# wsakobe/CylinderTag

Measured on AMD Instinct MI355X. Metric: frames/sec detect() 1920x1080, higher is better.
Workload: dtype u8; 1 GPU; synthetic 1920x1080 random-stripe frames, 4096 per step over 1 GPU(s), 4 planted CTag_2f12c markers each, detect(img,5,true,5), inputs resident in HBM; frames_per_gpu=4096, chunk=4096, parallelism=frames sharded, dp1, gather=none (1 GPU)

## Files before the change

cylindertag_amd/csrc/ctag_math.h:

```cpp
#pragma once
#include <stdint.h>

#if defined(__HIPCC__)
#define CTM_HD __host__ __device__ __forceinline__
#else
#define CTM_HD static inline
#endif

namespace ctm {

CTM_HD double bits_to_f64(uint64_t u) { double d; __builtin_memcpy(&d, &u, 8); return d; }
CTM_HD uint64_t f64_to_bits(double d) { uint64_t u; __builtin_memcpy(&u, &d, 8); return u; }
CTM_HD float bits_to_f32(uint32_t u) { float f; __builtin_memcpy(&f, &u, 4); return f; }
CTM_HD uint32_t f32_to_bits(float f) { uint32_t u; __builtin_memcpy(&u, &f, 4); return u; }

CTM_HD double fabs64(double x) { return bits_to_f64(f64_to_bits(x) & 0x7fffffffffffffffULL); }
CTM_HD float fabs32(float x) { return bits_to_f32(f32_to_bits(x) & 0x7fffffffu); }
CTM_HD bool isnan64(double x) { return x != x; }

CTM_HD double atan64(double x) {
    const double hi0 = 4.63647609000806093515e-01, hi1 = 7.85398163397448278999e-01,
                 hi2 = 9.82793723247329054082e-01, hi3 = 1.57079632679489655800e+00;
    const double lo0 = 2.26987774529616870924e-17, lo1 = 3.06161699786838301793e-17,
                 lo2 = 1.39033110312309984516e-17, lo3 = 6.12323399573676603587e-17;
// ... 102 lines not shown
    const int q = rem_pio2_64(x, &r);
    switch (q) {
        case 0: return ksin64(r);
        case 1: return kcos64(r);
        case 2: return -ksin64(r);
        default: return -kcos64(r);
    }
}
CTM_HD double cos64(double x) {
    if (fabs64(x) <= 7.85398163397448278999e-01) return kcos64(x);
    double r;
    const int q = rem_pio2_64(x, &r);
    switch (q) {
        case 0: return kcos64(r);
        case 1: return -ksin64(r);
        case 2: return -kcos64(r);
        default: return ksin64(r);
    }
}

CTM_HD void sincos64(double x, double* s, double* c) {
    double r = x;
    int q = 0;
    if (!(fabs64(x) <= 7.85398163397448278999e-01)) q = rem_pio2_64(x, &r);
    const double ks = ksin64(r), kc = kcos64(r);
    const double sv = (q & 1) ? kc : ks, cv = (q & 1) ? ks : kc;
    *s = (q & 2) ? -sv : sv;
    *c = ((q + 1) & 2) ? -cv : cv;
}

CTM_HD double exp64(double x) {
    const double T[32] = {
        1.00000000000000000e+00, 1.02189714865411663e+00, 1.04427378242741375e+00, 1.06714040067682370e+00,
        1.09050773266525769e+00, 1.11438674259589243e+00, 1.13878863475669156e+00, 1.16372485877757748e+00,
        1.18920711500272103e+00, 1.21524735998046896e+00, 1.24185781207348400e+00, 1.26905095719173322e+00,
        1.29683955465100964e+00, 1.32523664315974132e+00, 1.35425554693689265e+00, 1.38390988196383202e+00,
        1.41421356237309515e+00, 1.44518080697704665e+00, 1.47682614593949935e+00, 1.50916442759342284e+00,
        1.54221082540794074e+00, 1.57598084510788650e+00, 1.61049033194925428e+00, 1.64575547815396495e+00,
        1.68179283050742900e+00, 1.71861929812247793e+00, 1.75625216037329945e+00, 1.79470907500310717e+00,
        1.83400808640934243e+00, 1.87416763411029996e+00, 1.91520656139714740e+00, 1.95714412417540018e+00};
    const double inv = 4.61662413084468283841e+01;
    const double c_hi = 2.16608493865351192653e-02;
    const double c_lo = 5.96317165397058656257e-12;
    if (isnan64(x)) return x;
    if (x > 709.0) return bits_to_f64(0x7ff0000000000000ULL);
    if (x < -708.0) return 0.0;
    const double fn = __builtin_floor(x * inv + 0.5);
    const int n = (int)fn;
    const int j = n & 31, k = (n - j) / 32;
    const double r = (x - fn * c_hi) - fn * c_lo;
    double p = 1.3888888888888889e-03;
    p = p * r + 8.3333333333333332e-03;
    p = p * r + 4.1666666666666664e-02;
    p = p * r + 1.6666666666666666e-01;
    p = p * r + 0.5;
    p = p * r + 1.0;
    const double e = p * r + 1.0;
    const double scale = bits_to_f64((uint64_t)(k + 1023) << 52);
    return (T[j] * e) * scale;
}

CTM_HD double log64(double x) {
    const double ln2_hi = 6.93147180369123816490e-01, ln2_lo = 1.90821492927058770002e-10;
    const double Lg1 = 6.666666666666735130e-01, Lg2 = 3.999999999940941908e-01, Lg3 = 2.857142874366239149e-01,
                 Lg4 = 2.222219843214978396e-01, Lg5 = 1.818357216161805012e-01, Lg6 = 1.531383769920937332e-01,
                 Lg7 = 1.479819860511658591e-01;
    uint64_t u = f64_to_bits(x);
    uint32_t hx = (uint32_t)(u >> 32);
    int k = 0;
    if (hx < 0x00100000u || (hx >> 31)) {
        if ((u << 1) == 0) return -bits_to_f64(0x7ff0000000000000ULL);
        if (hx >> 31) return bits_to_f64(0x7ff8000000000000ULL);
        k -= 54;
        x = x * 18014398509481984.0;
        u = f64_to_bits(x);
        hx = (uint32_t)(u >> 32);
    } else if (hx >= 0x7ff00000u) {
        return x;
    } else if (u == 0x3ff0000000000000ULL) {
        return 0.0;
    }
    hx += 0x3ff00000u - 0x3fe6a09eu;
    k += (int)(hx >> 20) - 0x3ff;
    hx = (hx & 0x000fffffu) + 0x3fe6a09eu;
    const double f = bits_to_f64(((uint64_t)hx << 32) | (u & 0xffffffffULL)) - 1.0;
    const double hfsq = 0.5 * f * f;
    const double s = f / (2.0 + f);
    const double z = s * s;
    const double w = z * z;
    const double t1 = w * (Lg2 + w * (Lg4 + w * Lg6));
    const double t2 = z * (Lg1 + w * (Lg3 + w * (Lg5 + w * Lg7)));
    const double R = t2 + t1;
    const double dk = (double)k;
    return s * (hfsq + R) + dk * ln2_lo - hfsq + f + dk * ln2_hi;
}

CTM_HD double acos64(double t) {
    if (t >= 1.0) return 0.0;
    if (t <= -1.0) return 3.1415926535897931160E+00;
    return 2.0 * atan2_64(__builtin_sqrt(1.0 - t), __builtin_sqrt(1.0 + t));
}

constexpr float kAcosBelowTenMilli = 0.99995005130767822266f;

CTM_HD float atan2_32(float y, float x) { return (float)atan2_64((double)y, (double)x); }
CTM_HD float sin32(float x) { return (float)sin64((double)x); }
CTM_HD float cos32(float x) { return (float)cos64((double)x); }
CTM_HD void sincos32(float x, float* s, float* c) {
    double sd, cd;
    sincos64((double)x, &sd, &cd);
    *s = (float)sd;
    *c = (float)cd;
}
CTM_HD float exp32(float x) {
    if (x != x) return x;
    if (x < -87.0f) return 0.0f;
    if (x > 88.0f) return bits_to_f32(0x7f800000u);
    const float k = __builtin_rintf(x * 1.44269502162933349609375f);
    const float r = (x - k * 0.693145751953125f) - k * 1.428606765330187045037746429443359375e-06f;
    float p = 1.3933733571320772171020508e-03f;
    p = p * r + 8.3632357418537139892578125e-03f;
    p = p * r + 4.1666463017463684082031250e-02f;
    p = p * r + 1.6666576266288757324218750e-01f;
    p = p * r + 0.5f;
    const float e = (p * (r * r) + r) + 1.0f;
    return e * bits_to_f32((uint32_t)((int)k + 127) << 23);
}
CTM_HD float exp32_nonpos(float x) {
    if (x < -87.0f) return 0.0f;
    const float k = __builtin_rintf(x * 1.44269502162933349609375f);
    const float r = (x - k * 0.693145751953125f) - k * 1.428606765330187045037746429443359375e-06f;
    float p = 1.3933733571320772171020508e-03f;
    p = p * r + 8.3632357418537139892578125e-03f;
    p = p * r + 4.1666463017463684082031250e-02f;
    p = p * r + 1.6666576266288757324218750e-01f;
    p = p * r + 0.5f;
    const float e = (p * (r * r) + r) + 1.0f;
#if defined(__HIP_DEVICE_COMPILE__)
    return __builtin_amdgcn_ldexpf(e, (int)k);
#else
    return e * bits_to_f32((uint32_t)((int)k + 127) << 23);
#endif
}
CTM_HD bool exp32_k_is_zero(float x) { return x * 1.44269502162933349609375f >= -0.5f; }
CTM_HD float exp32_nonpos_k0(float x) {
    const float r = x;
    float p = 1.3933733571320772171020508e-03f;
    p = p * r + 8.3632357418537139892578125e-03f;
    p = p * r + 4.1666463017463684082031250e-02f;
    p = p * r + 1.6666576266288757324218750e-01f;
    p = p * r + 0.5f;
    return (p * (r * r) + r) + 1.0f;
}
struct Recip64 {
    double d, r;
};
CTM_HD Recip64 recip64(double d) {
    Recip64 R;
    R.d = d;
#if defined(__HIP_DEVICE_COMPILE__)
    double r = __builtin_amdgcn_rcp(d);
    r = __builtin_fma(r, __builtin_fma(-d, r, 1.0), r);
    r = __builtin_fma(r, __builtin_fma(-d, r, 1.0), r);
    R.r = r;
#else
    R.r = 0.0;
#endif
    return R;
}
CTM_HD double div64(double a, const Recip64& R) {
#if defined(__HIP_DEVICE_COMPILE__)
    const double q = a * R.r;
    return __builtin_fma(__builtin_fma(-R.d, q, a), R.r, q);
#else
    return a / R.d;
#endif
}
CTM_HD float sqrt32(float x) { return __builtin_sqrtf(x); }
CTM_HD double sqrt64(double x) { return __builtin_sqrt(x); }
CTM_HD float round32(float x) {
    const float ax = fabs32(x);
    if (!(ax < 8388608.0f)) return x;
    float r = __builtin_floorf(ax);
    if (ax - r >= 0.5f) r += 1.0f;
    return (f32_to_bits(x) >> 31) ? -r : r;
}

CTM_HD float fast_atan2_deg(float y, float x) {
    const float s = (float)(180.0 / 3.1415926535897932384626433832795);
    const float p1 = 0.9997878412794807f * s, p3 = -0.3258083974640975f * s,
                p5 = 0.1555786518463281f * s, p7 = -0.04432655554792128f * s;
    const float eps = (float)2.2204460492503131e-16;
    const float ax = fabs32(x), ay = fabs32(y);
    float a, c, c2;
    if (ax >= ay) {
        c = ay / (ax + eps);
        c2 = c * c;
        a = (((p7 * c2 + p5) * c2 + p3) * c2 + p1) * c;
    } else {
        c = ax / (ay + eps);
        c2 = c * c;
        a = 90.0f - (((p7 * c2 + p5) * c2 + p3) * c2 + p1) * c;
    }
    if (x < 0) a = 180.0f - a;
    if (y < 0) a = 360.0f - a;
    return a;
}

CTM_HD bool solve2x2(float a00, float a01, float a10, float a11, float b0, float b1, float& x0, float& x1) {
    double d = (double)a00 * a11 - (double)a01 * a10;
    if (d == 0.) return false;
    d = 1. / d;
    const float t = (float)(((double)b0 * a11 - (double)b1 * a01) * d);
    x1 = (float)(((double)b1 * a00 - (double)b0 * a10) * d);
    x0 = t;
    return true;
}

}
```

cylindertag_amd/csrc/k_quad.hip:

```cpp
#include "ctag_internal.h"
#include "ctag_math.h"
#include "ctag_wave.h"
#include <cstdio>
#include <type_traits>
#include <cstdlib>

namespace ctag {

struct QuadPtrs {
    const uint16_t* labels;
    const int32_t* tile_base;
    const int32_t* root_of;
    const int32_t* ncand;
    const Candidate* cand;
    QuadOut* quads;
    uint32_t* frame_flags;
    int32_t* line_count;
    int32_t* clp_used;
    uint32_t* cl_pool;
    LineDesc* line_desc;
    int32_t* line_sorted;
    int32_t* line_long;
    float* line_fit;
    CandAux* cand_aux;
    const uint8_t* pick_table;
    const uint16_t* pick_table16;
    const int32_t* pool_tile;
    const int32_t* member_head;
    const int32_t* member_next;
    int32_t* npacks;
    uint32_t* packs;
    uint32_t* pack_order;
    int32_t* npacks2;
    uint32_t* packs2;
    uint32_t* pack_order2;
    int32_t* npacks1;
    uint32_t* packs1;
    uint32_t* pack_order1;
    int32_t* ntotal1;
    unsigned long long* stamps;
    float thr_line, thr_expand, rac;
    int c2_far, c2_near;
    int cand_cap, line_cap;
    uint32_t cl_cap;
    float expand_eps;
    const uint64_t* mask;
    int mask_words;
};
static QuadPtrs quad_ptrs(const ChunkPlan& pl, const Workspace& ws, unsigned long long* stamps) {
    QuadPtrs P{};
    P.labels = ws.labels, P.tile_base = ws.tile_base, P.root_of = ws.root_of, P.ncand = ws.ncand, P.cand = ws.cand, P.quads = ws.quads, P.frame_flags = ws.frame_flags;
    P.line_count = ws.line_count, P.clp_used = ws.clp_used, P.cl_pool = ws.cl_pool, P.line_desc = ws.line_desc, P.line_sorted = ws.line_sorted, P.line_long = ws.line_long;
    P.line_fit = ws.line_fit, P.cand_aux = ws.cand_aux, P.pick_table = ws.pick_table, P.pick_table16 = ws.pick_table16;
    P.pool_tile = ws.pool_tile, P.member_head = ws.member_head, P.member_next = ws.member_next;
    P.npacks = ws.npacks, P.packs = ws.packs, P.pack_order = ws.pack_order, P.stamps = stamps;
    P.npacks2 = ws.npacks2, P.packs2 = ws.packs2, P.pack_order2 = ws.pack_order2;
    P.npacks1 = ws.npacks1, P.packs1 = ws.packs1, P.pack_order1 = ws.pack_order1, P.ntotal1 = ws.ntotal1;
    P.thr_line = ws.kp.thr_line, P.thr_expand = ws.kp.thr_expand, P.rac = ws.kp.rac, P.c2_far = ws.kp.c2_far, P.c2_near = ws.kp.c2_near, P.expand_eps = ws.kp.expand_eps;
    P.cand_cap = ws.cand_cap, P.line_cap = ws.line_cap, P.cl_cap = ws.cl_cap;
    P.mask = pl.fused ? reinterpret_cast<const uint64_t*>(ws.half) : nullptr, P.mask_words = ws.g.hcols >> 6;
    return P;
}

__device__ __forceinline__ uint32_t pack_xy(int x, int y) { return (uint32_t)x | ((uint32_t)y << 16); }
__device__ __forceinline__ int ux(uint32_t p) { return (int)(p & 0xffffu); }
__device__ __forceinline__ int uy(uint32_t p) { return (int)(p >> 16); }

__device__ __forceinline__ void moments_to_line(double x, double y, double x2, double y2, double xy, double w, float* line) {
    const ctm::Recip64 W = ctm::recip64(w);
    x = ctm::div64(x, W);
    y = ctm::div64(y, W);
    x2 = ctm::div64(x2, W);
    y2 = ctm::div64(y2, W);
    xy = ctm::div64(xy, W);
    const double dx2 = x2 - x * x, dy2 = y2 - y * y, dxy = xy - x * y;
    const float t = (float)ctm::atan2_64(2 * dxy, dx2 - dy2) / 2;
    double sn, cs;
    ctm::sincos64(t, &sn, &cs);
    line[0] = (float)cs;
    line[1] = (float)sn;
    line[2] = (float)x;
    line[3] = (float)y;
}

struct CvRng {
    uint64_t state;
    __device__ unsigned next() {
        state = (uint64_t)(unsigned)state * 4164903690U + (unsigned)(state >> 32);
        return (unsigned)state;
    }
};

#ifndef CTAG_WCAP
#define CTAG_WCAP 16
#endif
#ifndef CTAG_WUNROLL
#define CTAG_WUNROLL 2
#endif
#define CTAG_PRAGMA_(x) _Pragma(#x)
#define CTAG_PRAGMA(x) CTAG_PRAGMA_(x)
constexpr int kWCap = CTAG_WCAP;
struct GlobalPts {
    const uint32_t* p;
    __device__ __forceinline__ float2 operator()(int j) const {
        const uint32_t v = p[j];
        return make_float2((float)ux(v), (float)uy(v));
    }
};
struct LdsPts {
    const float2* p;
    __device__ __forceinline__ float2 operator()(int j) const { return p[j]; }
};
struct LdsPackedPts {
    const uint32_t* p;
    __device__ __forceinline__ float2 operator()(int j) const {
        const uint32_t v = p[j];
        return make_float2((float)ux(v), (float)uy(v));
    }
};
struct TablePicks {
    const uint8_t* t;
    __device__ __forceinline__ int operator()(int i) const { return t[i]; }
};
struct ListPicks {
    const uint16_t* t;
    __device__ __forceinline__ int operator()(int i) const { return t[i]; }
};
struct AllPicks {
    __device__ __forceinline__ int operator()(int i) const { return i; }
};
struct RestartResult {
    float line[4];
    double err;
};
__device__ __forceinline__ RestartResult restart_result(const float* res, int rstride) {
    RestartResult r;
    for (int q = 0; q < 4; q++) r.line[q] = res[q * rstride];
    const uint64_t lo = ctm::f32_to_bits(res[4 * rstride]), hi = ctm::f32_to_bits(res[5 * rstride]);
    r.err = ctm::bits_to_f64(lo | (hi << 32));
    return r;
}
template <class Pts, class Picks>
__device__ __forceinline__ void welsch_first_fit(const Pts pts, const Picks picks, int npick, float* line) {
    double x = 0, y = 0, x2 = 0, y2 = 0, xy = 0, w = 0;
    for (int i = 0; i < npick; i++) {
        const float2 p = pts(picks(i));
        const float px = p.x, py = p.y;
        x += px;
        y += py;
        x2 += px * px;
        y2 += py * py;
        xy += px * py;
        w += 1.f;
    }
    moments_to_line(x, y, x2, y2, xy, w, line);
}
struct WeightTrips {
    unsigned fast = 0, general = 0;
};
template <bool COUNT>
__device__ __forceinline__ float welsch_weight(float a, WeightTrips& trips) {
    const bool fast = wave_all(ctm::exp32_k_is_zero(a));
    if constexpr (COUNT) {
        const bool first = (int)__lane_id() == __ffsll((unsigned long long)__ballot(1)) - 1;
        trips.fast += first && fast ? 1u : 0u;
        trips.general += first && !fast ? 1u : 0u;
    }
    if (fast) return ctm::exp32_nonpos_k0(a);
    return ctm::exp32_nonpos(a);
}
template <int WS, bool COUNT, class Pts>
__device__ __forceinline__ bool welsch_rounds(const Pts pts, int n, double EPS, float* line, double& err, int it0, int it_stop, bool resume, float* wc, int ncache, WeightTrips& trips) {
    float prev[4] = {0.f, 0.f, 0.f, 0.f};
    const float c = 1 / 2.9846f;
#ifdef CTAG_WELSCH_MINERR_IN_LOOP
    double berr = 1.7976931348623157e308;
    float bl[4] = {0.f, 0.f, 0.f, 0.f};
#define CTAG_WELSCH_HAND_ON()       \
    do {                            \
        for (int q = 0; q < 4; q++) line[q] = bl[q]; \
        err = berr;                 \
    } while (0)
#else
#define CTAG_WELSCH_HAND_ON() do { } while (0)
#endif
    for (int it = it0; it < 30; it++) {
        if (it > 0 && !(resume && it == it0)) {
            const float t = line[0] * prev[0] + line[1] * prev[1];
            if (t >= ctm::kAcosBelowTenMilli) {
                const float dx = ctm::fabs32(line[2] - prev[2]);
                const float dy = ctm::fabs32(line[3] - prev[3]);
                const float d = dx > dy ? dx : dy;
                if (d < 0.01f) {
                    CTAG_WELSCH_HAND_ON();
                    return true;
                }
            }
        }
        if (it == it_stop) return false;
        const float lx = line[2], ly = line[3], nx = line[1], ny = -line[0];
        double sum_w = 0;
        err = 0;
        float2 pn0 = pts(min(0, n - 1));
        for (int j = 0; j < ncache; j++) {
            const float2 p = pn0;
            pn0 = pts(j + 1);
            const float x = p.x - lx, y = p.y - ly;
            const float r = ctm::fabs32(nx * x + ny * y);
            err += r;
            const float wj = welsch_weight<COUNT>(-r * r * c * c, trips);
            wc[j * WS] = wj;
            sum_w += wj;
        }
        float2 pn1 = pts(min(ncache, n - 1));
        for (int j = ncache; j < n; j++) {
            const float2 p = pn1;
            pn1 = pts(j + 1);
            const float x = p.x - lx, y = p.y - ly;
            const float r = ctm::fabs32(nx * x + ny * y);
            err += r;
            sum_w += welsch_weight<COUNT>(-r * r * c * c, trips);
        }
#ifdef CTAG_WELSCH_MINERR_IN_LOOP
        if (err < berr) {
            berr = err;
            for (int q = 0; q < 4; q++) bl[q] = line[q];
            if (err < EPS) return true;
        }
#else
        if (err < EPS) return true;
#endif
        double x = 0, y = 0, x2 = 0, y2 = 0, xy = 0, w = 0;
        if (ctm::fabs64(sum_w) > 1.1920928955078125e-07) {
            const double inv = 1. / sum_w;
            float2 pn2 = pts(min(0, n - 1));
            CTAG_PRAGMA(unroll CTAG_WUNROLL)
            for (int j = 0; j < ncache; j++) {
                const float2 p = pn2;
                pn2 = pts(j + 1);
                const float px = p.x, py = p.y;
                const float wj = (float)(wc[j * WS] * inv);
                x += wj * px;
                y += wj * py;
                x2 += wj * px * px;
                y2 += wj * py * py;
                xy += wj * px * py;
                w += wj;
            }
            float2 pn3 = pts(min(ncache, n - 1));
            for (int j = ncache; j < n; j++) {
                const float2 p = pn3;
                pn3 = pts(j + 1);
                const float px = p.x, py = p.y;
                const float r = ctm::fabs32(nx * (px - lx) + ny * (py - ly));
                const float wj = (float)(welsch_weight<COUNT>(-r * r * c * c, trips) * inv);
                x += wj * px;
                y += wj * py;
                x2 += wj * px * px;
                y2 += wj * py * py;
                xy += wj * px * py;
                w += wj;
            }
        } else {
            float2 pn4 = pts(min(0, n - 1));
            for (int j = 0; j < n; j++) {
                const float2 p = pn4;
                pn4 = pts(j + 1);
                const float px = p.x, py = p.y;
                x += px;
                y += py;
                x2 += px * px;
                y2 += py * py;
                xy += px * py;
                w += 1.f;
            }
        }
        prev[0] = line[0];
        prev[1] = line[1];
        prev[2] = line[2];
        prev[3] = line[3];
        moments_to_line(x, y, x2, y2, xy, w, line);
    }
    CTAG_WELSCH_HAND_ON();
    return true;
}
#undef CTAG_WELSCH_HAND_ON
__device__ __forceinline__ void restart_store(float* res, int rstride, const float* line, double err) {
    for (int q = 0; q < 4; q++) res[q * rstride] = line[q];
    const uint64_t eb = ctm::f64_to_bits(err);
    res[4 * rstride] = ctm::bits_to_f32((uint32_t)eb);
    res[5 * rstride] = ctm::bits_to_f32((uint32_t)(eb >> 32));
}
template <int WS, bool COUNT, class Pts, class Picks>
__device__ __forceinline__ void welsch_restart(const Pts pts, int n, const Picks picks, int npick, double EPS, float* res, int rstride, float* wc, WeightTrips& trips) {
    float line[4];
    double err = 0;
    welsch_first_fit(pts, picks, npick, line);
    (void)welsch_rounds<WS, COUNT>(pts, n, EPS, line, err, 0, 30, false, wc, min(n, kWCap), trips);
    restart_store(res, rstride, line, err);
}

#ifndef CTAG_PACK_WORDS
#define CTAG_PACK_WORDS 5120
#endif
#ifndef CTAG_PACK_WAVES
#define CTAG_PACK_WAVES 2
#endif
constexpr int kPackWords = CTAG_PACK_WORDS;
#ifndef CTAG_PACK_WAVES_P2
#define CTAG_PACK_WAVES_P2 4
#endif
constexpr int kPackWordsSmall = 2560, kPackWavesSmall = 4, kPackWavesSmallP2 = CTAG_PACK_WAVES_P2;
constexpr int kUnwind = 8;
constexpr int kWaveWords = 8192;
constexpr int kWaveWordsMax = 36864;
__host__ __device__ __forceinline__ int pack_points(int w, int h) { return min(2 * (w + h), w * h) + 1; }
__host__ __device__ __forceinline__ int pack_need(int w, int h) {
    const int C = pack_points(w, h);
    return ((w + 1) & ~1) + 2 * h + 2 * C + 4;
}
__host__ __device__ __forceinline__ int need2(int n) { return 2 * ((n + 1) & ~1); }
__host__ __device__ __forceinline__ int need1(int w, int h, int nt) { return (w + h + 2 * nt + 6) & ~1; }
constexpr int kScanWords = 2048;
__host__ __device__ __forceinline__ int scan_need(int w, int h) { return w + 3 * h + 4; }
constexpr int kMaskScanWords = 512, kMaskScanWordsLarge = 2048;
__host__ __device__ __forceinline__ int mask_scan_need(int w, int h) { return h * ((w + 31) / 32 + 1); }
__host__ __device__ __forceinline__ bool pack_big(int x_min, int w, int h, int big_points, int pack_words, int scan_words = 0) {
    (void)x_min;
    return pack_need(w, h) > pack_words || pack_points(w, h) > big_points || (scan_words > 0 && scan_need(w, h) > scan_words) ||
           (scan_words < 0 && mask_scan_need(w, h) > -scan_words);
}

struct CornerPre {
    float x, y, dis, ang;
};

__device__ __forceinline__ int pack_rank_sort(const int* s_key, uint16_t* s_ord, int n, int tid, int nt) {
    int neg = 0;
    for (int i = tid; i < n; i += nt) {
        const int ki = s_key[i];
        int rank = 0;
        for (int j = 0; j < n; j++) {
            const int kj = s_key[j];
            rank += (kj > ki || (kj == ki && j < i)) ? 1 : 0;
        }
        s_ord[rank] = (uint16_t)i;
        neg += ki < 0 ? 1 : 0;
    }
    return neg;
}
template <class KeyOf, class ValOf>
__device__ __forceinline__ int pack_counting_sort(int* s_cnt, uint32_t* out, int n, int tid, int nt, KeyOf key_of, ValOf val_of) {
    constexpr int kB = kLdsCand;
    auto bucket_of = [&](int key) { return key < 0 ? kB : kB - 1 - min(key, kB - 1); };
    for (int b = tid; b <= kB; b += nt) s_cnt[b] = 0;
    __syncthreads();
    for (int i = tid; i < n; i += nt) atomicAdd(&s_cnt[bucket_of(key_of(i))], 1);
    __syncthreads();
    if (tid == 0) {
        int run = 0;
        for (int b = 0; b <= kB; b++) {
            const int v = s_cnt[b];
            s_cnt[b] = run;
            run += v;
        }
        s_cnt[kB + 1] = run;
    }
    __syncthreads();
    const int first_neg = s_cnt[kB];
    __syncthreads();
    for (int i = tid; i < n; i += nt) out[atomicAdd(&s_cnt[bucket_of(key_of(i))], 1)] = val_of(i);
    __syncthreads();
    return first_neg;
}
template <class NeedOf>
__device__ __forceinline__ int build_packs(uint32_t* packs, int npacked, int max_per_pack, int pack_words, int tid, NeedOf need_of) {
    int np = 0, first = -1, cnt = 0, words = 0;
    for (int r0 = 0; r0 < npacked; r0 += 64) {
        const int r = r0 + tid;
        const int need = r < npacked ? need_of(r) : 0;
        const int m = min(64, npacked - r0);
        for (int k = 0; k < m; k++) {
            const int nk = __builtin_amdgcn_readlane(need, k);
            if (cnt > 0 && (cnt == max_per_pack || words + nk > pack_words)) {
                if (tid == 0) packs[np] = (uint32_t)first | ((uint32_t)cnt << 24);
                np++;
                cnt = 0;
                words = 0;
            }
            if (cnt == 0) first = r0 + k;
            cnt++;
            words += nk;
        }
    }
    if (cnt > 0) {
        if (tid == 0) packs[np] = (uint32_t)first | ((uint32_t)cnt << 24);
        np++;
    }
    return np;
}

__global__ __launch_bounds__(1024) void k_pack(QuadPtrs P, int nframes, int max_per_pack, int big_points, int pack_words, int scan_words) {
    __shared__ int s_key[kLdsCand + 2];
    __shared__ int s_need[kLdsCand];
    __shared__ uint16_t s_ord[kLdsCand];
    const int frame = blockIdx.x;
    if (frame >= nframes) return;
    const int tid = threadIdx.x, nt = blockDim.x;
    const int nc = min(P.ncand[frame], P.cand_cap);
    const Candidate* cand = P.cand + (size_t)frame * P.cand_cap;
    uint32_t* order = P.pack_order + (size_t)frame * P.cand_cap;
    uint32_t* packs = P.packs + (size_t)frame * P.cand_cap;
    auto key_of = [&](const Candidate& c) {
        const int w = c.x_max - c.x_min + 1, h = c.y_max - c.y_min + 1;
        return pack_big(c.x_min, w, h, big_points, pack_words, scan_words) ? -1 : pack_points(w, h);
    };
    auto slot_prefix = [&](int npacked, auto ci_of) {
        int base = 0;
        for (int r0 = 0; r0 < npacked; r0 += 64) {
            const int r = r0 + tid;
            int v = 0, ci = 0;
            if (r < npacked) {
                ci = ci_of(r);
                const Candidate c = cand[ci];
                v = pack_points(c.x_max - c.x_min + 1, c.y_max - c.y_min + 1) + 64;
            }
            int incl = v;
#pragma unroll
            for (int d = 1; d < 64; d <<= 1) {
                const int t = __shfl_up(incl, d, 64);
                if (tid >= d) incl += t;
            }
            if (r < npacked) P.cand_aux[(size_t)frame * P.cand_cap + ci].line0 = base + incl - v;
            base += __shfl(incl, 63, 64);
        }
        if (tid == 0) P.clp_used[frame] = base;
    };
    if (nc > kLdsCand) {
        const int first_big = pack_counting_sort(s_key, order, nc, tid, nt, [&](int i) { return key_of(cand[i]); }, [&](int i) { return (uint32_t)i; });
        if (tid >= 64) return;
        const int np = build_packs(packs, first_big, max_per_pack, pack_words, tid, [&](int r) {
            const Candidate c = cand[order[r]];
            return pack_need(c.x_max - c.x_min + 1, c.y_max - c.y_min + 1);
        });
        if (tid == 0) {
            P.npacks[2 * frame] = np;
            P.npacks[2 * frame + 1] = nc - first_big;
        }
        if (scan_words < 0) slot_prefix(first_big, [&](int r) { return (int)order[r]; });
        return;
    }
// ... 1582 lines not shown
            rank += (nj > ni || (nj == ni && j < i)) ? 1 : 0;
        }
        out[rank] = i;
    }
}

__device__ __forceinline__ void welsch_select(const QuadPtrs& P, int frame, int lid, int n, const float* res, int kstride, int rstride, int count) {
    const double EPS = n * 1.1920928955078125e-07;
    double min_err = 1.7976931348623157e308;
    float best[4] = {0.f, 0.f, 0.f, 0.f};
    for (int kk = 0; kk < count; kk++) {
        const RestartResult r = restart_result(res + kk * kstride, rstride);
        if (r.err < min_err) {
            min_err = r.err;
            for (int q = 0; q < 4; q++) best[q] = r.line[q];
#ifndef CTAG_WELSCH_MINERR_IN_LOOP
            if (r.err < EPS) break;
#endif
        }
    }
    float* o = P.line_fit + ((size_t)frame * P.line_cap + lid) * 4;
    for (int q = 0; q < 4; q++) o[q] = best[q];
}

#ifndef CTAG_WELSCH_BLOCK_WAVES
#define CTAG_WELSCH_BLOCK_WAVES 4
#endif
constexpr int kWB = CTAG_WELSCH_BLOCK_WAVES;
constexpr int kWT = kWB * 64;
constexpr int kWE = kWT / 20;
constexpr int kWRes = 10;
#ifdef CTAG_WELSCH_MINERR_IN_LOOP
#undef CTAG_WELSCH_REGROUP_AT
#define CTAG_WELSCH_REGROUP_AT 30
#endif
#ifndef CTAG_WELSCH_REGROUP_AT
#define CTAG_WELSCH_REGROUP_AT 2
#endif
constexpr int kWRegroupAt = CTAG_WELSCH_REGROUP_AT;
#ifndef CTAG_WPTS
#define CTAG_WPTS 128
#endif
constexpr int kWPts = CTAG_WPTS;
#ifndef CTAG_WPTSU
#define CTAG_WPTSU 240
#endif
constexpr int kWPtsU = CTAG_WPTSU;
static_assert(kWPtsU % 2 == 0 && kWPtsU < kPickN, "packed rows: an odd number of words, picks from the byte table");
static_assert(kWE * 20 <= kWT && kWCap >= kWRes + 6 && kWRes >= 5 && kWRes >= kWShort && kWPts < kPickN && kWE * kWPts * 8 >= kWT * 10 * 2 && (kWPts + 1) % 32 == 1, "k_welsch LDS layout");
struct WelschLds {
    float wc[kWCap * kWT];
    union {
    uint32_t ptu[kWE][kWPtsU + 1];
    float2 pt[kWE][kWPts + 1];
    };
    const uint32_t* gpts[kWE];
    int n[kWE];
    int lid[kWE];
    int cnt[kWB];
};

__device__ __forceinline__ void welsch_trips_add(const QuadPtrs& P, const WeightTrips& trips) {
    if (trips.fast) atomicAdd(&P.stamps[27], (unsigned long long)trips.fast);
    if (trips.general) atomicAdd(&P.stamps[28], (unsigned long long)trips.general);
}

template <int MODE, bool COUNT>
__device__ __forceinline__ void welsch_block_run(const QuadPtrs& P, WelschLds& S, int frame) {
    const int tid = threadIdx.x, lane = tid & 63, wave = tid >> 6;
    constexpr bool STAGED = MODE != 2;
    using PtsT = typename std::conditional<MODE == 0, LdsPts, typename std::conditional<MODE == 1, LdsPackedPts, GlobalPts>::type>::type;
    auto pts_of = [&](int e) -> PtsT {
        if constexpr (MODE == 0) return LdsPts{S.pt[e]};
        else if constexpr (MODE == 1) return LdsPackedPts{S.ptu[e]};
        else return GlobalPts{S.gpts[e]};
    };
    float line[4] = {0.f, 0.f, 0.f, 0.f};
    double err = 0;
    bool fin = true;
    int item = tid;
    WeightTrips trips;
    for (int phase = 0; phase < 2; phase++) {
        bool run;
        if (phase == 0) {
            run = tid < kWE * 20 && S.n[min(tid / 20, kWE - 1)] > 0;
            if (P.stamps) {
                const unsigned long long act = __ballot(run);
                if (lane == 0) atomicAdd(&P.stamps[24], (unsigned long long)__popcll(act));
            }
        } else {
            const unsigned long long bal = __ballot(!fin);
            if (lane == 0) S.cnt[wave] = __popcll(bal);
            __syncthreads();
            int base = 0, total = 0;
#pragma unroll
            for (int w = 0; w < kWB; w++) {
                const int c = S.cnt[w];
                base += w < wave ? c : 0;
                total += c;
            }
            if (!fin) {
                const int r = base + __popcll(bal & ((1ull << lane) - 1ull));
#pragma unroll
                for (int q = 0; q < 4; q++) S.wc[q * kWT + r] = line[q];
                S.wc[4 * kWT + r] = __int_as_float(tid);
            }
            __syncthreads();
            if (P.stamps && tid == 0) {
                atomicAdd(&P.stamps[25], (unsigned long long)total);
                atomicAdd(&P.stamps[26], 1ull);
            }
            run = tid < total;
            if (run) {
#pragma unroll
                for (int q = 0; q < 4; q++) line[q] = S.wc[q * kWT + tid];
                item = __float_as_int(S.wc[4 * kWT + tid]);
            }
        }
        if (run) {
            const int e = item / 20, k = item - e * 20;
            const int n = S.n[e];
            const double EPS = n * 1.1920928955078125e-07;
            const PtsT pts = pts_of(e);
            if (phase == 0) {
                if (STAGED || n < kPickN) {
                    welsch_first_fit(pts, TablePicks{P.pick_table + ((size_t)n * 20 + k) * 10}, min(n, 10), line);
                } else if (n < kPickN2) {
                    welsch_first_fit(pts, ListPicks{P.pick_table16 + ((size_t)(n - kPickN) * 20 + k) * 10}, 10, line);
                } else {
                    uint16_t* pk = reinterpret_cast<uint16_t*>(&S.pt[0][0]) + tid * 10;
                    CvRng rng;
                    rng.state = 0xffffffffffffffffULL;
                    for (int kk = 0; kk <= k; kk++) {
                        int got = 0;
                        while (got < 10) {
                            const int j = (int)(rng.next() % (unsigned)n);
                            bool dup = false;
                            for (int q = 0; q < got; q++) dup |= (pk[q] == j);
                            if (!dup) pk[got++] = (uint16_t)j;
                        }
                    }
                    for (int a = 1; a < 10; a++) {
                        const uint16_t v = pk[a];
                        int b = a - 1;
                        while (b >= 0 && pk[b] > v) {
                            pk[b + 1] = pk[b];
                            b--;
                        }
                        pk[b + 1] = v;
                    }
                    welsch_first_fit(pts, ListPicks{pk}, 10, line);
                }
            }
            fin = welsch_rounds<kWT, COUNT>(pts, n, EPS, line, err, phase == 0 ? 0 : kWRegroupAt, phase == 0 ? kWRegroupAt : 30, phase != 0, S.wc + tid, min(n, phase == 0 ? kWCap : kWRes), trips);
            if (fin) restart_store(S.wc + kWRes * kWT + item, kWT, line, err);
        } else {
            fin = true;
        }
    }
    if constexpr (COUNT) welsch_trips_add(P, trips);
    __syncthreads();
    if (tid < kWE && S.n[tid] > 0) welsch_select(P, frame, S.lid[tid], S.n[tid], S.wc + kWRes * kWT + tid * 20, 1, kWT, 20);
}

template <bool COUNT>
__device__ __forceinline__ void welsch_block(const QuadPtrs& P, WelschLds& S, int frame, int first, int L) {
    const int tid = threadIdx.x;
    if (tid < kWE) {
        int n = 0, lid = 0;
        const uint32_t* p = nullptr;
        if (first + tid < L) {
            lid = P.line_sorted[(size_t)frame * P.line_cap + first + tid];
            const LineDesc d = P.line_desc[(size_t)frame * P.line_cap + lid];
            n = d.n;
            p = P.cl_pool + (size_t)frame * P.cl_cap + d.off;
        }
        S.n[tid] = n;
        S.lid[tid] = lid;
        S.gpts[tid] = p;
    }
    __syncthreads();
    const int n0 = S.n[0];
    if (n0 <= kWPts) {
        for (int idx = tid; idx < kWE * kWPts; idx += kWT) {
            const int e = idx / kWPts, j = idx - e * kWPts;
            if (j < S.n[e]) {
                const uint32_t v = S.gpts[e][j];
                S.pt[e][j] = make_float2((float)ux(v), (float)uy(v));
            }
        }
        __syncthreads();
        welsch_block_run<0, COUNT>(P, S, frame);
    } else if (n0 <= kWPtsU) {
        for (int idx = tid; idx < kWE * kWPtsU; idx += kWT) {
            const int e = idx / kWPtsU, j = idx - e * kWPtsU;
            if (j < S.n[e]) S.ptu[e][j] = S.gpts[e][j];
        }
        __syncthreads();
        welsch_block_run<1, COUNT>(P, S, frame);
    } else {
        welsch_block_run<2, COUNT>(P, S, frame);
    }
}

template <bool COUNT>
__device__ __forceinline__ void welsch_short(const QuadPtrs& P, WelschLds& S, int frame, int first, int L) {
    const int tid = threadIdx.x;
    if (first + tid >= L) return;
    const int lid = P.line_sorted[(size_t)frame * P.line_cap + first + tid];
    const LineDesc d = P.line_desc[(size_t)frame * P.line_cap + lid];
    const int n = d.n;
    WeightTrips trips;
    welsch_restart<kWT, COUNT>(GlobalPts{P.cl_pool + (size_t)frame * P.cl_cap + d.off}, n, AllPicks{}, n, n * 1.1920928955078125e-07, S.wc + tid, kWT, S.wc + tid, trips);
    if constexpr (COUNT) welsch_trips_add(P, trips);
    welsch_select(P, frame, lid, n, S.wc + tid, 0, kWT, 1);
}

__device__ __forceinline__ bool welsch_lat_takes(const QuadPtrs& P, int frame, int L) {
    if (L > kLatLines) return false;
    if (L == 0) return true;
    const int longest = P.line_sorted[(size_t)frame * P.line_cap];
    return P.line_desc[(size_t)frame * P.line_cap + longest].n <= kLatPoints;
}

__device__ __forceinline__ double ordered_sum(double a, const float* src, int n) {
    int j = 0;
    for (; j + 8 <= n; j += 8) {
        float v[8];
#pragma unroll
        for (int u = 0; u < 8; u++) v[u] = src[j + u];
#pragma unroll
        for (int u = 0; u < 8; u++) a += v[u];
    }
    for (; j < n; j++) a += src[j];
    return a;
}

constexpr int kLatRankBlocks = 512;
constexpr int kLatChunk = 128;
static_assert(kLatPoints % kLatChunk == 0 && kLatChunk % 64 == 0, "k_welsch_lat: register / chunk layout");
#ifndef CTAG_WLAT_WAVES
#define CTAG_WLAT_WAVES 5
#endif
__global__ __launch_bounds__(64) __attribute__((amdgpu_waves_per_eu(CTAG_WLAT_WAVES))) void k_welsch_lat(QuadPtrs P, int nframes, float* rs) {
    constexpr int NQ = kLatPoints / 64, CQ = kLatChunk / 64, NC = kLatPoints / kLatChunk;
    __shared__ float s_r[kLatChunk], s_w[kLatChunk];
    __shared__ float s_t[6][kLatChunk];
    __shared__ double s_sum[8];
    __shared__ uint16_t s_pk[10];
    const int frame = blockIdx.z, k = blockIdx.x, lane = threadIdx.x;
    if (frame >= nframes) return;
    const int L = min(P.line_count[frame], P.line_cap);
    if (!welsch_lat_takes(P, frame, L)) return;
    const float c = 1 / 2.9846f;
    for (int rank = blockIdx.y; rank < L; rank += gridDim.y) {
        const unsigned long long dbg_t0 = P.stamps ? __builtin_amdgcn_s_memtime() : 0ull;
        __syncthreads();
        const int lid = P.line_sorted[(size_t)frame * P.line_cap + rank];
        const LineDesc d = P.line_desc[(size_t)frame * P.line_cap + lid];
        const int n = d.n;
        const uint32_t* pts = P.cl_pool + (size_t)frame * P.cl_cap + d.off;
        uint32_t pp[NQ];
        float ww[NQ];
#pragma unroll
        for (int q = 0; q < NQ; q++) {
            pp[q] = pts[min(lane + 64 * q, n - 1)];
            ww[q] = 0.f;
        }
        const int npick = min(n, 10);
        if (lane == 0) {
            if (n < kPickN) {
                const uint8_t* t = P.pick_table + ((size_t)n * 20 + k) * 10;
                for (int q = 0; q < npick; q++) s_pk[q] = t[q];
            } else if (n < kPickN2) {
                const uint16_t* t = P.pick_table16 + ((size_t)(n - kPickN) * 20 + k) * 10;
                for (int q = 0; q < npick; q++) s_pk[q] = t[q];
            } else {
                CvRng rng;
                rng.state = 0xffffffffffffffffULL;
                for (int kk = 0; kk <= k; kk++) {
                    int got = 0;
                    while (got < npick) {
                        const int j = (int)(rng.next() % (unsigned)n);
                        bool dup = false;
                        for (int q = 0; q < got; q++) dup |= (s_pk[q] == j);
                        if (!dup) s_pk[got++] = (uint16_t)j;
                    }
                }
                for (int a = 1; a < npick; a++) {
                    const uint16_t v = s_pk[a];
                    int b = a - 1;
                    while (b >= 0 && s_pk[b] > v) {
                        s_pk[b + 1] = s_pk[b];
                        b--;
                    }
                    s_pk[b + 1] = v;
                }
            }
        }
        __syncthreads();
        float line[4], prev[4] = {0.f, 0.f, 0.f, 0.f};
        {
            const uint32_t mine = pts[s_pk[lane < npick ? lane : 0]];
            double x = 0, y = 0, x2 = 0, y2 = 0, xy = 0, w = 0;
            for (int i = 0; i < npick; i++) {
                const uint32_t p = (uint32_t)__shfl((int)mine, i);
                const float fx = (float)ux(p), fy = (float)uy(p);
                x += fx;
                y += fy;
                x2 += fx * fx;
                y2 += fy * fy;
                xy += fx * fy;
                w += 1.f;
            }
            moments_to_line(x, y, x2, y2, xy, w, line);
        }
        const double EPS = n * 1.1920928955078125e-07;
        double err = 0;
#ifdef CTAG_WELSCH_MINERR_IN_LOOP
        double berr = 1.7976931348623157e308;
        float bl[4] = {0.f, 0.f, 0.f, 0.f};
#endif
        for (int it = 0; it < 30; it++) {
            if (it > 0) {
                const float t = line[0] * prev[0] + line[1] * prev[1];
// ... 441 lines not shown
```

Measured before the change: 278,700 frames/s.

## Restructure Welsch point loops into wave-uniform segments with unrolled bodies

Replaces the per-lane point loops in the Welsch line-fit rounds with a walker that splits iteration into segments bounded by the distinct per-lane point counts in the wave, found via ballot/readlane. Inside each segment every active lane runs the same trip count, and the body is unrolled by 4. The fast-exp test now compares |r| against a precomputed distance threshold instead of the scaled exponent argument, and |d| is widened to f64 with an abs modifier on the conversion. This is meant to cut divergence and loop overhead, at the cost of extra ballot/readlane scalar work and more code size and register pressure.

```diff
diff --git a/cylindertag_amd/csrc/ctag_math.h b/cylindertag_amd/csrc/ctag_math.h
--- a/cylindertag_amd/csrc/ctag_math.h
+++ b/cylindertag_amd/csrc/ctag_math.h
@@ -278,6 +278,8 @@
     p = p * r + 0.5f;
     return (p * (r * r) + r) + 1.0f;
 }
+constexpr float kWelschK0MaxDist = 1.75704896450042724609375f;
+CTM_HD bool welsch_k_is_zero(float abs_r) { return abs_r <= kWelschK0MaxDist; }
 struct Recip64 {
     double d, r;
 };
diff --git a/cylindertag_amd/csrc/k_quad.hip b/cylindertag_amd/csrc/k_quad.hip
--- a/cylindertag_amd/csrc/k_quad.hip
+++ b/cylindertag_amd/csrc/k_quad.hip
@@ -94,11 +94,6 @@
 #ifndef CTAG_WCAP
 #define CTAG_WCAP 16
 #endif
-#ifndef CTAG_WUNROLL
-#define CTAG_WUNROLL 2
-#endif
-#define CTAG_PRAGMA_(x) _Pragma(#x)
-#define CTAG_PRAGMA(x) CTAG_PRAGMA_(x)
 constexpr int kWCap = CTAG_WCAP;
 struct GlobalPts {
     const uint32_t* p;
@@ -158,9 +153,11 @@
 struct WeightTrips {
     unsigned fast = 0, general = 0;
 };
+constexpr float kWelschC = 1 / 2.9846f;
 template <bool COUNT>
-__device__ __forceinline__ float welsch_weight(float a, WeightTrips& trips) {
-    const bool fast = wave_all(ctm::exp32_k_is_zero(a));
+__device__ __forceinline__ float welsch_weight(float r, WeightTrips& trips) {
+    const float a = -r * r * kWelschC * kWelschC;
+    const bool fast = wave_all(ctm::welsch_k_is_zero(r));
     if constexpr (COUNT) {
         const bool first = (int)__lane_id() == __ffsll((unsigned long long)__ballot(1)) - 1;
         trips.fast += first && fast ? 1u : 0u;
@@ -169,10 +166,79 @@
     if (fast) return ctm::exp32_nonpos_k0(a);
     return ctm::exp32_nonpos(a);
 }
+
+__device__ __forceinline__ double welsch_abs_f64(float d) {
+    double r;
+    asm("v_cvt_f64_f32_e64 %0, |%1|" : "=v"(r) : "v"(d));
+    return r;
+}
+
+constexpr int kWStops = 8;
+struct WelschStops {
+    int s[kWStops];
+    bool ok;
+    __device__ __forceinline__ int next_after(int j0) const {
+        int m = 0x7fffffff;
+#pragma unroll
+        for (int q = 0; q < kWStops; q++) m = s[q] > j0 && s[q] < m ? s[q] : m;
+        return m;
+    }
+};
+__device__ __forceinline__ WelschStops welsch_stops(int n) {
+    WelschStops st;
+    unsigned long long todo = __ballot(1);
+#pragma unroll
+    for (int q = 0; q < kWStops; q++) {
+        int v = 0;
+        if (todo != 0ull) {
+            v = __builtin_amdgcn_readlane(n, __ffsll(todo) - 1);
+            todo &= ~__ballot(n == v);
+        }
+        st.s[q] = v;
+    }
+    st.ok = todo == 0ull;
+    return st;
+}
+__device__ __forceinline__ int welsch_next_stop(int n, int j0) {
+    int m = 0x7fffffff;
+    for (unsigned long long todo = __ballot(n > j0); todo != 0ull;) {
+        const int v = __builtin_amdgcn_readlane(n, __ffsll(todo) - 1);
+        m = min(m, v);
+        todo &= ~__ballot(n == v);
+    }
+    return m;
+}
+template <class Pts, class Body>
+__device__ __forceinline__ void welsch_walk(const WelschStops& st, const Pts pts, int n, int lo, int cap, Body body) {
+    float2 pn = make_float2(0.f, 0.f);
+    if (n > lo) pn = pts(lo);
+    int j0 = lo;
+    while (j0 < cap && __ballot(n > j0) != 0ull) {
+        const int stop = min(st.ok ? st.next_after(j0) : welsch_next_stop(n, j0), cap);
+        if (n > j0) {
+            int j = j0;
+            for (; j + 4 <= stop; j += 4) {
+#pragma unroll
+                for (int u = 0; u < 4; u++) {
+                    const float2 p = pn;
+                    pn = pts(j + u + 1);
+                    body(j + u, p);
+                }
+            }
+            for (; j < stop; j++) {
+                const float2 p = pn;
+                pn = pts(j + 1);
+                body(j, p);
+            }
+        }
+        j0 = stop;
+    }
+}
 template <int WS, bool COUNT, class Pts>
-__device__ __forceinline__ bool welsch_rounds(const Pts pts, int n, double EPS, float* line, double& err, int it0, int it_stop, bool resume, float* wc, int ncache, WeightTrips& trips) {
+__device__ __forceinline__ bool welsch_rounds(const Pts pts, int n, double EPS, float* line, double& err, int it0, int it_stop, bool resume, float* wc, int wcap, WeightTrips& trips) {
     float prev[4] = {0.f, 0.f, 0.f, 0.f};
-    const float c = 1 / 2.9846f;
+    const WelschStops st = welsch_stops(n);
+    constexpr int kNoCap = 0x7fffffff;
 #ifdef CTAG_WELSCH_MINERR_IN_LOOP
     double berr = 1.7976931348623157e308;
     float bl[4] = {0.f, 0.f, 0.f, 0.f};
@@ -201,26 +267,20 @@
         const float lx = line[2], ly = line[3], nx = line[1], ny = -line[0];
         double sum_w = 0;
         err = 0;
-        float2 pn0 = pts(min(0, n - 1));
-        for (int j = 0; j < ncache; j++) {
-            const float2 p = pn0;
-            pn0 = pts(j + 1);
+        welsch_walk(st, pts, n, 0, wcap, [&](int j, float2 p) __attribute__((always_inline)) {
             const float x = p.x - lx, y = p.y - ly;
-            const float r = ctm::fabs32(nx * x + ny * y);
-            err += r;
-            const float wj = welsch_weight<COUNT>(-r * r * c * c, trips);
+            const float d = nx * x + ny * y, r = __builtin_fabsf(d);
+            err += welsch_abs_f64(d);
+            const float wj = welsch_weight<COUNT>(r, trips);
             wc[j * WS] = wj;
             sum_w += wj;
-        }
-        float2 pn1 = pts(min(ncache, n - 1));
-        for (int j = ncache; j < n; j++) {
-            const float2 p = pn1;
-            pn1 = pts(j + 1);
+        });
+        welsch_walk(st, pts, n, wcap, kNoCap, [&](int j, float2 p) __attribute__((always_inline)) {
             const float x = p.x - lx, y = p.y - ly;
-            const float r = ctm::fabs32(nx * x + ny * y);
-            err += r;
-            sum_w += welsch_weight<COUNT>(-r * r * c * c, trips);
-        }
+            const float d = nx * x + ny * y, r = __builtin_fabsf(d);
+            err += welsch_abs_f64(d);
+            sum_w += welsch_weight<COUNT>(r, trips);
+        });
 #ifdef CTAG_WELSCH_MINERR_IN_LOOP
         if (err < berr) {
             berr = err;
@@ -233,11 +293,7 @@
         double x = 0, y = 0, x2 = 0, y2 = 0, xy = 0, w = 0;
         if (ctm::fabs64(sum_w) > 1.1920928955078125e-07) {
             const double inv = 1. / sum_w;
-            float2 pn2 = pts(min(0, n - 1));
-            CTAG_PRAGMA(unroll CTAG_WUNROLL)
-            for (int j = 0; j < ncache; j++) {
-                const float2 p = pn2;
-                pn2 = pts(j + 1);
+            welsch_walk(st, pts, n, 0, wcap, [&](int j, float2 p) __attribute__((always_inline)) {
                 const float px = p.x, py = p.y;
                 const float wj = (float)(wc[j * WS] * inv);
                 x += wj * px;
@@ -246,26 +302,20 @@
                 y2 += wj * py * py;
                 xy += wj * px * py;
                 w += wj;
-            }
-            float2 pn3 = pts(min(ncache, n - 1));
-            for (int j = ncache; j < n; j++) {
-                const float2 p = pn3;
-                pn3 = pts(j + 1);
+            });
+            welsch_walk(st, pts, n, wcap, kNoCap, [&](int j, float2 p) __attribute__((always_inline)) {
                 const float px = p.x, py = p.y;
-                const float r = ctm::fabs32(nx * (px - lx) + ny * (py - ly));
-                const float wj = (float)(welsch_weight<COUNT>(-r * r * c * c, trips) * inv);
+                const float r = __builtin_fabsf(nx * (px - lx) + ny * (py - ly));
+                const float wj = (float)(welsch_weight<COUNT>(r, trips) * inv);
                 x += wj * px;
                 y += wj * py;
                 x2 += wj * px * px;
                 y2 += wj * py * py;
                 xy += wj * px * py;
                 w += wj;
-            }
+            });
         } else {
-            float2 pn4 = pts(min(0, n - 1));
-            for (int j = 0; j < n; j++) {
-                const float2 p = pn4;
-                pn4 = pts(j + 1);
+            welsch_walk(st, pts, n, 0, kNoCap, [&](int j, float2 p) __attribute__((always_inline)) {
                 const float px = p.x, py = p.y;
                 x += px;
                 y += py;
@@ -273,7 +323,7 @@
                 y2 += py * py;
                 xy += px * py;
                 w += 1.f;
-            }
+            });
         }
         prev[0] = line[0];
         prev[1] = line[1];
@@ -296,7 +346,7 @@
     float line[4];
     double err = 0;
     welsch_first_fit(pts, picks, npick, line);
-    (void)welsch_rounds<WS, COUNT>(pts, n, EPS, line, err, 0, 30, false, wc, min(n, kWCap), trips);
+    (void)welsch_rounds<WS, COUNT>(pts, n, EPS, line, err, 0, 30, false, wc, kWCap, trips);
     restart_store(res, rstride, line, err);
 }
 
@@ -2185,7 +2235,7 @@
                     welsch_first_fit(pts, ListPicks{pk}, 10, line);
                 }
             }
-            fin = welsch_rounds<kWT, COUNT>(pts, n, EPS, line, err, phase == 0 ? 0 : kWRegroupAt, phase == 0 ? kWRegroupAt : 30, phase != 0, S.wc + tid, min(n, phase == 0 ? kWCap : kWRes), trips);
+            fin = welsch_rounds<kWT, COUNT>(pts, n, EPS, line, err, phase == 0 ? 0 : kWRegroupAt, phase == 0 ? kWRegroupAt : 30, phase != 0, S.wc + tid, phase == 0 ? kWCap : kWRes, trips);
             if (fin) restart_store(S.wc + kWRes * kWT + item, kWT, line, err);
         } else {
             fin = true;
@@ -2203,7 +2253,9 @@
         int n = 0, lid = 0;
         const uint32_t* p = nullptr;
         if (first + tid < L) {
-            lid = P.line_sorted[(size_t)frame * P.line_cap + first + tid];
+            int rank = first + tid;
+            asm volatile("" : "+v"(rank));
+            lid = P.line_sorted[(size_t)frame * P.line_cap + rank];
             const LineDesc d = P.line_desc[(size_t)frame * P.line_cap + lid];
             n = d.n;
             p = P.cl_pool + (size_t)frame * P.cl_cap + d.off;
```

After: 282,800 frames/s (median of 6 runs). 1.02x the previous value.
